# mpc001/auto_avsr

Measured on AMD Instinct MI355X. Metric: video-frames/sec/node (25fps 88x88, max-frames=1600), E2E training step (fwd+bwd+clip+AdamW), higher is better.
Workload: dtype f16 activations x f16x2 weights (atrunk3, atrunk4, decoder, encoder, trunk3, trunk4) + split-bf16 (everything else) forward / bf16 backward

## Files before the change

### auto_avsr_amd/csrc/gemm_core.h

```cpp
#pragma once
#include <algorithm>
#include "prims.h"

namespace avsr_gemm_impl {

struct Params {
    const void* A;
    const void* B;
    const void* B2;
    int lda, ldb;
    int M, N, K;
    int k_chunk;
    const float* bias;
    int act;
    const void* gate;
    int gate_dtype, ldg;
    float gate_scale;
    float drop_p;
    uint64_t seed;
    float alpha;
    const float* alpha_dev;
    const uint64_t* seed_dev;
    const float* resid;
    int ldr;
    void* C;
    void* C2;
    int ldc2;
    int c_dtype, ldc;
    int accumulate;
    int nsplit, batch_h, nbatch;
    long sAb, sAh, sBb, sBh, sCb, sCh;
    int a_skew, skew_off, skew_lim;
    int resid_dtype;
    int cH, cW, cC;
    int cOH, cOW;
    int cKH, cKW, cS, cPH, cPW;
    int cT, cKT, cPT;
    float* colsum;
    float* colstat;
    int colstat_rows;
    float* colsum_a;
    int cN, xcd_order, ncls;
    int k_rot;
    int cls_tile0[5], cls_py[4], cls_px[4], cls_y0[4], cls_x0[4], cls_h[4], cls_w[4], cls_nkh[4], cls_nkw[4];
};

template <class T> struct Raw8;
template <> struct Raw8<bf16_t> {
    bf16x8 v;
    AVSR_DEV void zero() { v = bf16x8{0, 0, 0, 0, 0, 0, 0, 0}; }
    AVSR_DEV void load(const bf16_t* p) { v = *reinterpret_cast<const bf16x8*>(p); }
    AVSR_DEV void set(int e, const bf16_t* p) { v[e] = (short)*p; }
    AVSR_DEV float get(int e) const { return bf2f((bf16_t)v[e]); }
};
template <> struct Raw8<float> {
    f32x4 a, b;
    AVSR_DEV void zero() { a = f32x4{0, 0, 0, 0}; b = a; }
    AVSR_DEV void load(const float* p) {
        a = *reinterpret_cast<const f32x4*>(p);
        b = *reinterpret_cast<const f32x4*>(p + 4);
    }
    AVSR_DEV void set(int e, const float* p) {
        if (e < 4) a[e] = *p; else b[e - 4] = *p;
    }
    AVSR_DEV float get(int e) const { return e < 4 ? a[e] : b[e - 4]; }
};

template <class T>
AVSR_DEV Raw8<T> load_chunk(const T* base, int ld, int r, int c, int r_lim, int c_lim) {
    Raw8<T> out;
    if (r < r_lim && c + 8 <= c_lim) {
        out.load(base + (size_t)r * ld + c);
    } else {
        out.zero();
        if (r < r_lim) {
            for (int e = 0; e < 8; e++)
                if (c + e < c_lim) out.set(e, base + (size_t)r * ld + c + e);
        }
    }
    return out;
}

template <class T>
AVSR_DEV Raw8<T> load_chunk_skew(const T* base, int ld, int r, int c, int r_lim, int m_lim, int off, int lim) {
    Raw8<T> out;
    out.zero();
    if (r < r_lim) {
        for (int e = 0; e < 8; e++) {
            const int j = c + e + r - off;
            if (c + e < m_lim && j >= 0 && j < lim) out.set(e, base + (size_t)r * ld + j);
        }
    }
    return out;
}

template <int TM, int TN>
AVSR_DEV void epilogue(f32x16 (&acc)[TM][TN], const Params& p, int row0, int col0, int lane, int zs, long c_off) {
    const float inv_keep = p.drop_p > 0.f ? 1.0f / (1.0f - p.drop_p) : 1.0f;
    const float alpha = p.alpha * (p.alpha_dev ? *p.alpha_dev : 1.f);
    const uint64_t seed = p.seed + (p.seed_dev ? *p.seed_dev : 0ull);
#pragma unroll
    for (int i = 0; i < TM; i++)
#pragma unroll
        for (int j = 0; j < TN; j++) {
            const int col = col0 + j * 32 + (lane & 31);
            if (col >= p.N) continue;
            const float bias = (p.bias && zs == 0) ? p.bias[col] : 0.f;
#pragma unroll
            for (int r = 0; r < 16; r++) {
                const int row = row0 + i * 32 + (r & 3) + 8 * (r >> 2) + 4 * (lane >> 5);
                if (row >= p.M) continue;
                float v = acc[i][j][r] + bias;
                if (p.act == 1) v = fmaxf(v, 0.f);
                else if (p.act == 2) v = avsr_silu(v);
                if (p.gate) {
                    const float g = p.gate_dtype == 0
                                        ? reinterpret_cast<const float*>(p.gate)[(size_t)row * p.ldg + col]
                                        : bf2f(reinterpret_cast<const bf16_t*>(p.gate)[(size_t)row * p.ldg + col]);
                    v = g > 0.f ? v * p.gate_scale : 0.f;
                }
                if (p.drop_p > 0.f)
                    v *= dropout_scale(seed, (uint64_t)row * (uint64_t)p.N + col, p.drop_p, inv_keep);
                v *= alpha;
                if (p.resid && zs == 0)
                    v += p.resid_dtype == 0 ? p.resid[(size_t)row * p.ldr + col]
                                            : bf2f(reinterpret_cast<const bf16_t*>(p.resid)[(size_t)row * p.ldr + col]);
                if (p.c_dtype == 0) {
                    float* c = reinterpret_cast<float*>(p.C) + c_off + (size_t)row * p.ldc + col;
// ... 494 lines not shown
```

### auto_avsr_amd/csrc/gemm_fast.hip

```cpp
#include "gemm_fast_kernel.h"
#include "gemm_pair.h"
#include "avsr_hip.h"

namespace {

using avsr_gemm_impl::Params;

#define g_tune avsr_tune_knobs

using avsr_fast::FastKernel;

template <int BM, int BN, int STAGES, int CV, int WGM, int WGN, int ABL, int KS, int F16 = 0, int WP = 1>
__global__ __launch_bounds__(64 * WGM * WGN * KS) void gemm_fast_kernel(Params p) {
    AVSR_DYN_SMEM(smem);
    FastKernel<BM, BN, STAGES, CV, WGM, WGN, ABL, KS, F16, WP>::run(p, smem);
}

template <int BM, int BN, int STAGES, int CV = 0, int WGM = 2, int WGN = 2, int ABL = 0, int KS = 1, int F16 = 0, int WP = 1>
void launch_fast(Params& p, int split_k, hipStream_t stream) {
    using K = FastKernel<BM, BN, STAGES, CV, WGM, WGN, ABL, KS, F16, WP>;
    p.k_rot = CV == 0 ? g_tune[7] : 0;
    p.xcd_order = g_tune[1] == 0 ? (CV == 0 && BM == 64 && BN == 64) : (g_tune[1] == 1);
    int gy;
    if (CV == 0) {
        int kc = (p.K + split_k - 1) / split_k;
        kc = ((kc + 63) / 64) * 64;
        split_k = (p.K + kc - 1) / kc;
        p.k_chunk = kc;
        gy = (p.M + BM - 1) / BM;
    } else {
        split_k = 1;
        int t0 = 0;
        for (int c = 0; c < p.ncls; c++) {
            p.cls_tile0[c] = t0;
            t0 += (int)(((long)p.cN * p.cls_h[c] * p.cls_w[c] + BM - 1) / BM);
        }
        p.cls_tile0[p.ncls] = t0;
        gy = t0;
    }
    dim3 grid((p.N + BN - 1) / BN, gy, split_k), block(K::NTHR);
    AVSR_LAUNCH((gemm_fast_kernel<BM, BN, STAGES, CV, WGM, WGN, ABL, KS, F16, WP>), grid, block, K::LDS_BYTES, stream, p);
}

template <int CV>
bool launch_tile(int tile, Params& p, int split_k, hipStream_t stream) {
    switch (tile) {
        case 1: if (CV == 0) { launch_fast<64, 64, 3, 0>(p, split_k, stream); return true; } return false;
        case 2: launch_fast<128, 64, 3, CV>(p, split_k, stream); return true;
        case 3:
            if (CV == 1 && g_tune[2] == 1) launch_fast<128, 128, 3, 1, 2, 2, 1>(p, split_k, stream);
            else if (CV == 1 && g_tune[2] == 2) launch_fast<128, 128, 3, 1, 2, 2, 2>(p, split_k, stream);
            else launch_fast<128, 128, 3, CV>(p, split_k, stream);
            return true;
        case 4: launch_fast<128, 128, 2, CV>(p, split_k, stream); return true;
        case 5: launch_fast<256, 128, 3, CV, 4, 2>(p, split_k, stream); return true;
        case 6: launch_fast<256, 128, 3, CV, 2, 2>(p, split_k, stream); return true;
        case 7: launch_fast<128, 64, 2, CV>(p, split_k, stream); return true;
        case 8: launch_fast<256, 64, 3, CV, 4, 2>(p, split_k, stream); return true;
        case 9: if (CV == 0) { launch_fast<64, 64, 5, 0>(p, split_k, stream); return true; } return false;
        case 10: if (CV == 0) { launch_fast<64, 64, 8, 0>(p, split_k, stream); return true; } return false;
        case 11: if (CV == 0) { launch_fast<128, 64, 4, 0>(p, split_k, stream); return true; } return false;
        case 12: if (CV == 0) { launch_fast<128, 64, 6, 0>(p, split_k, stream); return true; } return false;
        case 13: if (CV == 0) { launch_fast<128, 128, 4, 0>(p, split_k, stream); return true; } return false;
        case 14: if (CV == 0) { launch_fast<64, 64, 3, 0, 2, 2, 1>(p, split_k, stream); return true; } return false;
        case 15: if (CV == 0) { launch_fast<64, 64, 3, 0, 2, 2, 2>(p, split_k, stream); return true; } return false;
        case 16: if (CV == 0) { launch_fast<64, 64, 3, 0, 2, 2, 0, 2>(p, split_k, stream); return true; } return false;
        case 17: if (CV == 0) { launch_fast<128, 64, 3, 0, 2, 2, 0, 2>(p, split_k, stream); return true; } return false;
        case 18: if (CV == 0) { launch_fast<128, 128, 3, 0, 2, 2, 0, 2>(p, split_k, stream); return true; } return false;
        default: return false;
    }
}

template <int CV>
bool launch_tile_h16(int tile, Params& p, int split_k, hipStream_t stream) {
    switch (tile) {
        case 1: if (CV == 0) { launch_fast<64, 64, 3, 0, 2, 2, 0, 1, 1>(p, split_k, stream); return true; } return false;
        case 4: launch_fast<128, 128, 2, CV, 2, 2, 0, 1, 1>(p, split_k, stream); return true;
        case 7: launch_fast<128, 64, 2, CV, 2, 2, 0, 1, 1>(p, split_k, stream); return true;
        default: return false;
    }
}

template <int CV>
bool launch_tile_h16x2(int tile, Params& p, int split_k, hipStream_t stream) {
    switch (tile) {
        case 1: if (CV == 0) { launch_fast<64, 64, 3, 0, 2, 2, 0, 1, 1, 2>(p, split_k, stream); return true; } return false;
        case 21: if (CV == 0) { launch_fast<64, 64, 2, 0, 2, 2, 0, 1, 1, 2>(p, split_k, stream); return true; } return false;
        case 4: launch_fast<128, 128, 2, CV, 2, 2, 0, 1, 1, 2>(p, split_k, stream); return true;
        case 7: launch_fast<128, 64, 2, CV, 2, 2, 0, 1, 1, 2>(p, split_k, stream); return true;
        case 2: launch_fast<128, 64, 3, CV, 2, 2, 0, 1, 1, 2>(p, split_k, stream); return true;
        case 5: launch_fast<256, 128, 2, CV, 4, 2, 0, 1, 1, 2>(p, split_k, stream); return true;
        case 8: launch_fast<256, 64, 2, CV, 4, 2, 0, 1, 1, 2>(p, split_k, stream); return true;
        case 22: launch_fast<128, 128, 2, CV, 2, 4, 0, 1, 1, 2>(p, split_k, stream); return true;
        case 23: launch_fast<256, 64, 3, CV, 4, 2, 0, 1, 1, 2>(p, split_k, stream); return true;
        case 31: if (CV == 0) { launch_fast<64, 64, 3, 0, 2, 2, 1, 1, 1, 2>(p, split_k, stream); return true; } return false;
        case 32: if (CV == 0) { launch_fast<64, 64, 3, 0, 2, 2, 2, 1, 1, 2>(p, split_k, stream); return true; } return false;
        case 33: if (CV == 0) { launch_fast<128, 64, 2, 0, 2, 2, 1, 1, 1, 2>(p, split_k, stream); return true; } return false;
        case 34: if (CV == 0) { launch_fast<128, 64, 2, 0, 2, 2, 2, 1, 1, 2>(p, split_k, stream); return true; } return false;
        case 35: if (CV == 0) { launch_fast<256, 128, 2, 0, 4, 2, 1, 1, 1, 2>(p, split_k, stream); return true; } return false;
        case 36: if (CV == 0) { launch_fast<256, 128, 2, 0, 4, 2, 2, 1, 1, 2>(p, split_k, stream); return true; } return false;
        default: return false;
    }
}

}

int avsr_conv_patch_supported(int N, int H, int W, int Cg, int Cout_eff, int KH, int KW, int stride, int pad_h, int pad_w);
int avsr_conv_patch_launch(int mode, const void* src, const void* w, const void* w_lo, int ldw, const void* resid, void* out, void* out2,
                           const void* zero_page, int N, int H, int W, int Cg, int Cout_eff, hipStream_t stream);
int avsr_conv3x3_c64_supported(int H, int W);
int avsr_conv3x3_c64_launch(int flip, const void* src, const void* wq, const void* resid, void* out, const void* zero_page, int N,
                            int H, int W, hipStream_t stream);

static int gemm16_nt_impl(int f16, const void* A, int lda, const void* B, const void* B_lo, int ldb, int M, int N, int K, const float* bias,
                          int act, const void* gate, int gate_dtype, int ldg, float gate_scale, float drop_p,
                          uint64_t seed, const uint64_t* seed_dev, float alpha, const float* alpha_dev,
                          const void* resid, int resid_dtype, int ldr, void* C, int c_dtype, int ldc, int accumulate,
                          int split_k, int tile, float* colsum, void* c2, int ldc2, hipStream_t stream) {
    AVSR_REQUIRE(!(colsum && accumulate), "gemm_bf16_nt: colsum needs a non-accumulating output");
    AVSR_REQUIRE(K > 0 && K % 64 == 0, "gemm_bf16_nt: K must be a positive multiple of 64");
    AVSR_REQUIRE(lda % 8 == 0 && ldb % 8 == 0, "gemm_bf16_nt: lda/ldb must be multiples of 8 elements");
    AVSR_REQUIRE(((uintptr_t)A % 16) == 0 && ((uintptr_t)B % 16) == 0, "gemm_bf16_nt: operands must be 16-byte aligned");
    AVSR_REQUIRE(!(accumulate && c_dtype != 0), "gemm_bf16_nt: accumulate needs an f32 output");
// ... 371 lines not shown
```

### auto_avsr_amd/csrc/gemm_fast_kernel.h

```cpp
#pragma once
#include <type_traits>
#include "gemm_core.h"

namespace avsr_fast {

using avsr_gemm_impl::Params;

template <int BM, int BN, int STAGES, int CV = 0, int WGM = 2, int WGN = 2, int ABL = 0, int KS = 1, int F16 = 0, int WP = 1>
struct FastKernel {
    static_assert(WP == 1 || (WP == 2 && F16 == 1 && KS == 1), "two weight planes: f16 operands only");
    static constexpr int BK = 64, NQ = WGM * WGN, NW = NQ * KS, NTHR = 64 * NW;
    static constexpr int KPG = (BK / 16) / KS;
    static_assert(KS == 1 || KS == 2 || KS == 4, "k-split of the 64-wide tile");
    static constexpr int WM = BM / WGM, WN = BN / WGN, TM = WM / 32, TN = WN / 32;
    static constexpr int A_BYTES = BM * 128, B_BYTES = BN * 128, STAGE_BYTES = A_BYTES + WP * B_BYTES;
    static constexpr int A_LOADS = BM / (8 * NW), B_LOADS = BN / (8 * NW);
    static constexpr int LPT = A_LOADS + WP * B_LOADS;
    static constexpr size_t RING_BYTES = (size_t)STAGES * STAGE_BYTES, EPI_BYTES = (size_t)BM * (BN + 4) * 4;
    static constexpr size_t MAP_OFF = RING_BYTES > EPI_BYTES ? RING_BYTES : EPI_BYTES;
    static constexpr size_t LDS_BYTES = MAP_OFF + (CV == 2 ? BM * 4 : 0);
    static_assert(A_LOADS >= 1 && B_LOADS >= 1 && BM % (8 * NW) == 0 && BN % (8 * NW) == 0, "tile / wave-count mismatch");
    static_assert(WM % 32 == 0 && WN % 32 == 0, "wave tile must be a multiple of 32x32");

    struct Rows {
// ... 30 lines not shown
            if (CV == 0) {
                const int gr = min(m0 + r, p.M - 1);
                ri.a[i] = A + (size_t)gr * p.lda + c * 8;
                ri.mask[i] = 0;
            } else {
                int n, a, b;
                row_coords(p, cls, m0 + r, n, a, b);
                int ya, xa;
                if (CV == 1) {
                    ya = a * p.cS - p.cPH;
                    xa = b * p.cS - p.cPW;
                } else {
                    ya = (p.cls_y0[cls] + a * p.cS + p.cPH) / p.cS;
                    xa = (p.cls_x0[cls] + b * p.cS + p.cPW) / p.cS;
                }
                ri.a[i] = A + ((long)n * p.cH * p.cW + (long)ya * p.cW + xa) * p.cC + c * 8;
                uint32_t mk = 0;
                for (int t = 0; t < tp.ntaps; t++) {
                    const int ta = t / tp.nkw, tb = t - ta * tp.nkw;
                    const int y = CV == 1 ? ya + ta : ya - ta, x = CV == 1 ? xa + tb : xa - tb;
                    if (y >= 0 && y < p.cH && x >= 0 && x < p.cW) mk |= 1u << t;
                }
                ri.mask[i] = mk;
            }
        }
#pragma unroll
        for (int i = 0; i < B_LOADS; i++) {
            const int r = (wave * B_LOADS + i) * 8 + rsub;
            const int c = pc ^ ((r >> 1) & 7);
            const int gr = min(n0 + r, p.N - 1);
            ri.b[i] = B + (size_t)gr * p.ldb + c * 8;
        }
        return ri;
    }

    static AVSR_DEV void issue(const Params& p, const Rows& ri, const Taps& tp, int kbeg, int t, char* stage, int wave,
                               int rot = 0, int nt = 1) {
        long da, db;
        int tap = 0;
        if (CV == 0) {
            int tt = t + rot;
            if (tt >= nt) tt -= nt;
            da = db = kbeg + tt * BK;
        } else {
            tap = t / tp.cpt;
            const int cb = (t - tap * tp.cpt) * BK;
            const int ta = tap / tp.nkw, tb = tap - ta * tp.nkw;
            if (CV == 1) {
                da = (long)(ta * p.cW + tb) * p.cC + cb;
                db = (long)tap * p.cC + cb;
            } else {
                da = -(long)(ta * p.cW + tb) * p.cC + cb;
                db = (long)((tp.py + ta * p.cS) * p.cKW + tp.px + tb * p.cS) * p.cC + cb;
            }
        }
#pragma unroll
        for (int i = 0; i < A_LOADS; i++) {
            const bf16_t* src = ri.a[i] + da;
            if (CV != 0) src = ((ri.mask[i] >> tap) & 1u) ? src : reinterpret_cast<const bf16_t*>(p.gate);
            glds16(src, stage + (wave * A_LOADS + i) * 1024);
        }
#pragma unroll
        for (int i = 0; i < B_LOADS; i++) glds16(ri.b[i] + db, stage + A_BYTES + (wave * B_LOADS + i) * 1024);
        if (WP == 2) {
            const long lo = reinterpret_cast<const bf16_t*>(p.B2) - reinterpret_cast<const bf16_t*>(p.B);
#pragma unroll
            for (int i = 0; i < B_LOADS; i++) glds16(ri.b[i] + db + lo, stage + A_BYTES + B_BYTES + (wave * B_LOADS + i) * 1024);
        }
    }

    static AVSR_DEV bf16x8 frag(const char* base, int r, int chunk) {
        return *reinterpret_cast<const bf16x8*>(base + r * 128 + ((chunk ^ ((r >> 1) & 7)) << 4));
    }

    static AVSR_DEV void run(const Params& p, char* smem) {
        run_at(p, smem, blockIdx.x, blockIdx.y, blockIdx.z, gridDim.x, gridDim.y, gridDim.z);
    }
    static AVSR_DEV void run_at(const Params& p, char* smem, int bx, int by, int bz, int gx_, int gy_, int gz_) {
        const bf16_t* A = reinterpret_cast<const bf16_t*>(p.A);
        const bf16_t* B = reinterpret_cast<const bf16_t*>(p.B);
        const int lane = threadIdx.x & 63, wave = wave_id();
        const int kg = wave / NQ, wq = wave - kg * NQ;
        const int wm = wq / WGN, wn = wq % WGN;
        if (p.xcd_order && gz_ == 1) {
            const int gx = gx_, total = gx * gy_;
            const int id = by * gx + bx;
            const int xcd = id & 7, slot = id >> 3, q = total >> 3, r = total & 7;
            const int nid = (xcd < r ? xcd * (q + 1) : r * (q + 1) + (xcd - r) * q) + slot;
            by = nid / gx;
            bx = nid - by * gx;
        }
        const int n0 = bx * BN;
        const int zs = bz;

        int cls = 0, m0 = by * BM, nt, kbeg = 0;
        Taps tp{1, 1, 1, 0, 0};
        if (CV == 0) {
            kbeg = zs * p.k_chunk;
            nt = (min(p.K, kbeg + p.k_chunk) - kbeg) / BK;
        } else {
            while (cls + 1 < p.ncls && by >= p.cls_tile0[cls + 1]) cls++;
            m0 = (by - p.cls_tile0[cls]) * BM;
            tp.nkw = p.cls_nkw[cls];
            tp.ntaps = p.cls_nkh[cls] * tp.nkw;
            tp.cpt = p.cC / BK;
            tp.py = p.cls_py[cls];
            tp.px = p.cls_px[cls];
            nt = tp.ntaps * tp.cpt;
        }
        int* rowmap = nullptr;
        if (CV == 2) {
            rowmap = reinterpret_cast<int*>(smem + MAP_OFF);
            for (int r = threadIdx.x; r < BM; r += NTHR) {
                int n, a, b;
                const bool ok = row_coords(p, cls, m0 + r, n, a, b);
                rowmap[r] = ok ? (n * p.cOH + p.cls_y0[cls] + a * p.cS) * p.cOW + p.cls_x0[cls] + b * p.cS : -1;
            }
        }

        f32x16 acc[TM][TN];
        f32x16 acc_lo[WP == 2 ? TM : 1][WP == 2 ? TN : 1];
#pragma unroll
        for (int i = 0; i < TM; i++)
#pragma unroll
            for (int j = 0; j < TN; j++)
#pragma unroll
                for (int r = 0; r < 16; r++) {
                    acc[i][j][r] = 0.f;
                    if (WP == 2) acc_lo[i][j][r] = 0.f;
                }

        const Rows ri = decode_rows(p, A, B, m0, n0, cls, tp, wave, lane);
        const int rot = (CV == 0 && p.k_rot) ? (int)(((unsigned)(by * gx_ + bx) * (unsigned)p.k_rot) % (unsigned)nt) : 0;
#pragma unroll
        for (int s = 0; s < STAGES - 1; s++)
            if (s < nt) issue(p, ri, tp, kbeg, s, smem + s * STAGE_BYTES, wave, rot, nt);

        auto step = [&](int t, auto issue_flag) {
            constexpr bool ISSUE = decltype(issue_flag)::value;
            if (ISSUE) {
                wait_vmcnt<(STAGES - 2) * LPT>();
            } else {
                switch (nt - 1 - t) {
                    case 0: wait_vmcnt<0>(); break;
                    default: wait_vmcnt<(STAGES > 2 ? LPT : 0)>(); break;
                }
            }
            block_barrier_raw();
            const char* As = smem + (t % STAGES) * STAGE_BYTES;
            const char* Bs = As + A_BYTES;
            bf16x8 fa[2][TM], fb[2][TN], fl[2][WP == 2 ? TN : 1];
            const int arow = wm * WM + (lane & 31), brow = wn * WN + (lane & 31);
            auto load_frags = [&](int set, int ks) {
                const int chunk = ks * 2 + (lane >> 5);
#pragma unroll
                for (int i = 0; i < TM; i++) fa[set][i] = frag(As, arow + i * 32, chunk);
#pragma unroll
                for (int j = 0; j < TN; j++) fb[set][j] = frag(Bs, brow + j * 32, chunk);
                if (WP == 2) {
#pragma unroll
                    for (int j = 0; j < TN; j++) fl[set][j] = frag(Bs + B_BYTES, brow + j * 32, chunk);
                }
            };
            const int ks0 = kg * KPG;
            if (ABL != 1) {
                load_frags(0, ks0);
                if (KPG > 1) load_frags(1, ks0 + 1);
// ... 42 lines not shown
```

### auto_avsr_amd/csrc/gemm_pair.hip

```cpp
#include "gemm_fast_kernel.h"
#include "gemm_tn_kernel.h"
#include "gemm_pair.h"
#include "avsr_hip.h"

namespace {

using avsr_gemm_impl::Params;
using avsr_fast::FastKernel;
using Tn = avsr_tn::TnKernel<3, 0>;
using Tn4 = avsr_tn::TnKernel<3, 0, 1, 1, 4>;
using Tn128 = avsr_tn::TnKernel<2, 0, 2, 2>;

struct PairState {
    bool active = false, have_nt = false, have_tn = false;
    Params nt, tn;
    int nt_tile = 0;
    int gxa = 0, gya = 0;
    int gxb = 0, gyb = 0, gzb = 0;
    int tn_big = 0;
    hipStream_t stream = nullptr;
};
thread_local PairState g_pair;

template <class KA, class KB>
__global__ __launch_bounds__(256) void gemm_pair_kernel(Params pa, Params pb, int na, int gxa, int gya, int gxb, int gyb) {
    AVSR_DYN_SMEM(smem);
    int b = blockIdx.x;
    if (b < na) {
        const int by = b / gxa;
        KA::run_at(pa, smem, b - by * gxa, by, 0, gxa, gya, 1);
    } else {
        b -= na;
        const int r = b / gxb;
        KB::run_at(pb, smem, b - r * gxb, r % gyb, r / gyb);
    }
}

template <class KA, class KB>
void launch_pair(const PairState& s) {
    const int na = s.have_nt ? s.gxa * s.gya : 0;
    const int nb = s.have_tn ? s.gxb * s.gyb * s.gzb : 0;
    const size_t lds = KA::LDS_BYTES > KB::LDS_BYTES ? KA::LDS_BYTES : KB::LDS_BYTES;
    AVSR_LAUNCH((gemm_pair_kernel<KA, KB>), dim3(na + nb), dim3(256), lds, s.stream, s.nt, s.tn, na, s.gxa > 0 ? s.gxa : 1,
                s.gya > 0 ? s.gya : 1, s.gxb > 0 ? s.gxb : 1, s.gyb > 0 ? s.gyb : 1);
}

}

namespace avsr_pair {

bool stash_nt(const Params& p, int tile, int split_k, hipStream_t stream) {
    PairState& s = g_pair;
    if (!s.active || s.have_nt || split_k > 1 || p.accumulate || (tile != 1 && tile != 7)) return false;
    if (s.have_tn && s.stream != stream) return false;
    s.nt = p;
    s.nt.xcd_order = (tile == 1 && avsr_tune_knobs[1] != 2) ? 1 : 0;
    s.nt.k_chunk = ((p.K + 63) / 64) * 64;
    s.nt_tile = tile;
    const int BM = tile == 1 ? 64 : 128;
    s.gxa = (p.N + 63) / 64;
    s.gya = (p.M + BM - 1) / BM;
    s.stream = stream;
    s.have_nt = true;
    return true;
}

bool stash_tn(const Params& p, int split_k, hipStream_t stream) {
    PairState& s = g_pair;
    if (!s.active || s.have_tn) return false;
    if (s.have_nt && s.stream != stream) return false;
    if (split_k < 1) split_k = 1;
    int kc = (p.K + split_k - 1) / split_k;
    kc = ((kc + 63) / 64) * 64;
    split_k = (p.K + kc - 1) / kc;
    s.tn = p;
    s.tn_big = avsr_tune_knobs[19] == 2 && p.M >= 128 && p.N >= 128;
    if (s.tn_big) {
        split_k = 1;
        kc = ((p.K + 63) / 64) * 64;
    }
    const int tb = s.tn_big ? 128 : 64;
    s.tn.k_chunk = kc;
    s.gxb = (p.N + tb - 1) / tb;
    s.gyb = (p.M + tb - 1) / tb;
    s.gzb = split_k;
    s.stream = stream;
    s.have_tn = true;
    return true;
}

}

extern "C" int avsr_gemm_pair_begin(void) {
    AVSR_REQUIRE(!g_pair.active, "gemm_pair_begin: a pair is already open on this thread");
    g_pair = PairState{};
    g_pair.active = true;
    return 0;
}

extern "C" int avsr_gemm_pair_end(void) {
    PairState s = g_pair;
    g_pair = PairState{};
    AVSR_REQUIRE(s.active, "gemm_pair_end: no open pair on this thread");
    if (!s.have_nt && !s.have_tn) return 0;
    if (s.tn_big) {
        if (s.have_nt && s.nt_tile == 7) launch_pair<FastKernel<128, 64, 2, 0>, Tn128>(s);
        else launch_pair<FastKernel<64, 64, 3, 0>, Tn128>(s);
    } else if (avsr_tune_knobs[20] == 1) {
        if (s.have_nt && s.nt_tile == 7) launch_pair<FastKernel<128, 64, 2, 0>, Tn4>(s);
        else launch_pair<FastKernel<64, 64, 3, 0>, Tn4>(s);
    } else if (s.have_nt && s.nt_tile == 7) launch_pair<FastKernel<128, 64, 2, 0>, Tn>(s);
    else launch_pair<FastKernel<64, 64, 3, 0>, Tn>(s);
    AVSR_CHECK_LAUNCH("gemm_pair");
    return 0;
}
```

### auto_avsr_amd/csrc/gemm_tn_fast.hip

```cpp
#include "gemm_tn_kernel.h"
#include "gemm_pair.h"
#include "avsr_hip.h"

namespace {

using avsr_gemm_impl::Params;

using avsr_tn::TnKernel;

template <int STAGES, int CV>
__global__ __launch_bounds__(256) void gemm_tn_fast_kernel(Params p) {
    AVSR_DYN_SMEM(smem);
    TnKernel<STAGES, CV>::run(p, smem);
}

template <int CV>
void launch_tn(Params& p, int split_k, hipStream_t stream) {
    if (split_k < 1) split_k = 1;
    int kc = (p.K + split_k - 1) / split_k;
    kc = ((kc + 63) / 64) * 64;
    split_k = (p.K + kc - 1) / kc;
    p.k_chunk = kc;
    dim3 grid((p.N + 63) / 64, (p.M + 63) / 64, split_k), block(256);
    AVSR_LAUNCH((gemm_tn_fast_kernel<3, CV>), grid, block, (TnKernel<3, CV>::LDS_BYTES), stream, p);
}

}

extern "C" int avsr_gemm_bf16_tn(const void* A, int lda, const void* B, int ldb, int M, int N, int K, float* C, int ldc,
                                 int accumulate, int split_k, const void* zero_page, float* colsum_a, hipStream_t stream) {
    AVSR_REQUIRE(lda % 8 == 0 && ldb % 8 == 0 && M % 8 == 0 && N % 8 == 0, "gemm_bf16_tn: M, N, lda, ldb must be multiples of 8");
    AVSR_REQUIRE(((uintptr_t)A % 16) == 0 && ((uintptr_t)B % 16) == 0, "gemm_bf16_tn: operands must be 16-byte aligned");
    AVSR_REQUIRE(zero_page != nullptr, "gemm_bf16_tn: zero page required");
    AVSR_REQUIRE(!(split_k > 1 && !accumulate), "gemm_bf16_tn: split-K needs accumulate=1");
    if (M <= 0 || N <= 0 || K <= 0) return 0;
    Params p{};
    p.A = A; p.B = B; p.lda = lda; p.ldb = ldb; p.M = M; p.N = N; p.K = K;
    p.alpha = 1.f; p.gate_scale = 1.f; p.gate = zero_page;
    p.C = C; p.c_dtype = 0; p.ldc = ldc; p.accumulate = accumulate;
    p.colsum_a = colsum_a;
    p.nsplit = 1; p.batch_h = 1; p.nbatch = 1;
    if (avsr_det()) {
        p.colsum_a = nullptr;
        launch_tn<0>(p, 1, stream);
        if (colsum_a) avsr_colsum_det(A, 1, lda, K, M, colsum_a, stream);
        AVSR_CHECK_LAUNCH("gemm_bf16_tn");
        return 0;
    }
    if (avsr_pair::stash_tn(p, split_k, stream)) return 0;
    launch_tn<0>(p, split_k, stream);
    AVSR_CHECK_LAUNCH("gemm_bf16_tn");
    return 0;
}

extern "C" int avsr_conv2d_wgrad_bf16(const void* dy, const void* x, float* dwp, const void* zero_page, int N, int H, int W,
                                      int Cin, int Cout, int KH, int KW, int stride, int pad_h, int pad_w,
                                      hipStream_t stream) {
    AVSR_REQUIRE(Cin % 64 == 0 && Cout % 8 == 0, "conv2d_wgrad_bf16: Cin must be a multiple of 64, Cout of 8");
    AVSR_REQUIRE(zero_page != nullptr, "conv2d_wgrad_bf16: zero page required");
    const int OH = (H + 2 * pad_h - KH) / stride + 1, OW = (W + 2 * pad_w - KW) / stride + 1;
    if (N <= 0) return 0;
    Params p{};
    p.A = dy; p.B = x; p.lda = Cout; p.ldb = Cin;
    p.M = Cout; p.N = KH * KW * Cin; p.K = N * OH * OW;
    p.alpha = 1.f; p.gate_scale = 1.f; p.gate = zero_page;
    p.C = dwp; p.c_dtype = 0; p.ldc = p.N; p.accumulate = 1;
    p.nsplit = 1; p.batch_h = 1; p.nbatch = 1;
    p.cH = H; p.cW = W; p.cC = Cin; p.cOH = OH; p.cOW = OW; p.cKH = KH; p.cKW = KW; p.cS = stride; p.cPH = pad_h; p.cPW = pad_w;
    p.cT = 1; p.cKT = 1;
    const long tiles = (long)((p.M + 63) / 64) * ((p.N + 63) / 64);
    const long target = avsr_tune_knobs[24] > 0 ? avsr_tune_knobs[24] : (tiles <= 12 ? 512 : (tiles >= 96 ? 2048 : 1024));
    long split = target / (tiles < 1 ? 1 : tiles);
    if (split > p.K / 512) split = p.K / 512;
    if (split < 1 || avsr_det()) split = 1;
    launch_tn<3>(p, (int)split, stream);
    AVSR_CHECK_LAUNCH("conv2d_wgrad_bf16");
    return 0;
}
```

### auto_avsr_amd/csrc/gemm_tn_kernel.h

```cpp
#pragma once
#include "gemm_core.h"

namespace avsr_tn {

using avsr_gemm_impl::Params;

template <int STAGES, int CV, int TMS = 1, int TNS = 1, int DEPTH = 2>
struct TnKernel {
    static_assert(DEPTH == 2 || DEPTH == 4, "fragment pipeline depth");
    static_assert(CV == 0 || (TMS == 1 && TNS == 1), "gathered B operand: 64 x 64 tiles only");
    static constexpr int BM = 64 * TMS, BN = 64 * TNS, BK = 64;
    static constexpr int OP_BYTES = BK * 128;
    static constexpr int A_BYTES = TMS * OP_BYTES, STAGE_BYTES = (TMS + TNS) * OP_BYTES;
    static constexpr int LPT = 2 * (TMS + TNS);
    static constexpr size_t RING_BYTES = (size_t)STAGES * STAGE_BYTES, EPI_BYTES = (size_t)BM * (BN + 4) * 4;
    static constexpr size_t LDS_BYTES = RING_BYTES > EPI_BYTES ? RING_BYTES : EPI_BYTES;

    static AVSR_DEV void issue(const Params& p, const bf16_t* A, const bf16_t* B, int m0, int n0, int k0, int kend,
                               char* stage, int wave, int lane) {
        const int ksub = lane >> 3, chunk = (lane & 7) * 8;
        const bf16_t* zero = reinterpret_cast<const bf16_t*>(p.gate);
        int kh = 0, kw = 0, cbase = 0;
        if (CV == 3) {
            const int tap = n0 / p.cC;
            cbase = n0 - tap * p.cC;
            kh = tap / p.cKW;
            kw = tap - kh * p.cKW;
        }
#pragma unroll
        for (int i = 0; i < 2; i++) {
            const int kr = (wave * 2 + i) * 8 + ksub;
            const int k = k0 + kr;
            const bool kin = k < kend;
#pragma unroll
            for (int s = 0; s < TMS; s++) {
                const int mc = m0 + s * 64 + chunk;
                const bf16_t* sa = (kin && mc < p.M) ? A + (size_t)k * p.lda + mc : zero;
                glds16(sa, stage + s * OP_BYTES + (wave * 2 + i) * 1024);
            }
#pragma unroll
            for (int s = 0; s < TNS; s++) {
                const bf16_t* sb = zero;
                if (CV == 0) {
                    const int nc = n0 + s * 64 + chunk;
                    if (kin && nc < p.N) sb = B + (size_t)k * p.ldb + nc;
                } else if (kin) {
                    const int pix = p.cOH * p.cOW;
                    const int n = k / pix, r = k - n * pix;
                    const int oh = r / p.cOW, ow = r - oh * p.cOW;
                    const int ih = oh * p.cS + kh - p.cPH, iw = ow * p.cS + kw - p.cPW;
                    if (ih >= 0 && ih < p.cH && iw >= 0 && iw < p.cW)
                        sb = B + (((size_t)n * p.cH + ih) * p.cW + iw) * p.cC + cbase + chunk;
                }
                glds16(sb, stage + A_BYTES + s * OP_BYTES + (wave * 2 + i) * 1024);
            }
        }
    }

    static AVSR_DEV void frag_async(const char* base, int c0, int ks, int lane, bf16x4& lo, bf16x4& hi) {
        const int g = lane >> 4, i = lane & 15;
        const bf16_t* t = reinterpret_cast<const bf16_t*>(base);
        const int row = ks * 16 + 8 * (g >> 1) + (i >> 2);
        const int col = c0 + 16 * (g & 1) + 4 * (i & 3);
        lo = lds_tr16_async(t + row * 64 + col);
        hi = lds_tr16_async(t + (row + 4) * 64 + col);
    }

    static AVSR_DEV void run(const Params& p, char* smem) { run_at(p, smem, blockIdx.x, blockIdx.y, blockIdx.z); }
    static AVSR_DEV void run_at(const Params& p, char* smem, int bx, int by, int bz) {
        const bf16_t* A = reinterpret_cast<const bf16_t*>(p.A);
        const bf16_t* B = reinterpret_cast<const bf16_t*>(p.B);
        const int lane = threadIdx.x & 63, wave = wave_id();
        const int wm = wave >> 1, wn = wave & 1;
        const int m0 = by * BM, n0 = bx * BN;
        const int zs = bz;
        const int kbeg = zs * p.k_chunk;
        const int kend = min(p.K, kbeg + p.k_chunk);
        const int nt = (kend - kbeg + BK - 1) / BK;
        f32x16 acc[TMS][TNS];
#pragma unroll
        for (int i = 0; i < TMS; i++)
#pragma unroll
            for (int j = 0; j < TNS; j++)
#pragma unroll
                for (int r = 0; r < 16; r++) acc[i][j][r] = 0.f;
        const bool do_cs = CV == 0 && p.colsum_a != nullptr && bx == 0;
        float cs[TMS];
#pragma unroll
        for (int s = 0; s < TMS; s++) cs[s] = 0.f;
#pragma unroll
        for (int s = 0; s < STAGES - 1; s++)
            if (s < nt) issue(p, A, B, m0, n0, kbeg + s * BK, kend, smem + s * STAGE_BYTES, wave, lane);
        constexpr int NF = 2 * (TMS + TNS);
        for (int t = 0; t < nt; t++) {
            const int later = min(STAGES - 2, nt - 1 - t);
            if (later >= 1) wait_vmcnt<LPT>(); else wait_vmcnt<0>();
            block_barrier_raw();
            if (t + STAGES - 1 < nt)
                issue(p, A, B, m0, n0, kbeg + (t + STAGES - 1) * BK, kend, smem + ((t + STAGES - 1) % STAGES) * STAGE_BYTES,
                      wave, lane);
            const char* As = smem + (t % STAGES) * STAGE_BYTES;
            const char* Bs = As + A_BYTES;
            if (do_cs) {
#pragma unroll
                for (int s = 0; s < TMS; s++) {
                    const bf16_t* col = reinterpret_cast<const bf16_t*>(As + s * OP_BYTES) + (wave * 16) * 64 + lane;
#pragma unroll
                    for (int r = 0; r < 16; r++) cs[s] += bf2f(col[r * 64]);
                }
            }
            bf16x4 fa[DEPTH][TMS][2], fb[DEPTH][TNS][2];
            auto request = [&](int set, int ks) {
#pragma unroll
                for (int i = 0; i < TMS; i++) {
                    const int col = wm * 32 * TMS + 32 * i;
                    frag_async(As + (col >> 6) * OP_BYTES, col & 63, ks, lane, fa[set][i][0], fa[set][i][1]);
                }
#pragma unroll
                for (int j = 0; j < TNS; j++) {
                    const int col = wn * 32 * TNS + 32 * j;
                    frag_async(Bs + (col >> 6) * OP_BYTES, col & 63, ks, lane, fb[set][j][0], fb[set][j][1]);
                }
            };
            request(0, 0);
            if (DEPTH == 4) {
#pragma unroll
                for (int ks = 1; ks < BK / 16; ks++) request(ks, ks);
            }
#pragma unroll
            for (int ks = 0; ks < BK / 16; ks++) {
                const int c = DEPTH == 4 ? ks : (ks & 1);
                if (DEPTH == 4) {
                    switch (ks) {
                        case 0: lds_wait<3 * NF>(); break;
                        case 1: lds_wait<2 * NF>(); break;
                        case 2: lds_wait<NF>(); break;
                        default: lds_wait<0>(); break;
                    }
                } else if (ks + 1 < BK / 16) {
                    request(c ^ 1, ks + 1);
                    lds_wait<NF>();
                } else {
                    lds_wait<0>();
                }
                bf16x8 a[TMS], b[TNS];
#pragma unroll
                for (int i = 0; i < TMS; i++) {
                    lds_tie(fa[c][i][0]);
                    lds_tie(fa[c][i][1]);
                    a[i] = bf16x8{fa[c][i][0][0], fa[c][i][0][1], fa[c][i][0][2], fa[c][i][0][3],
                                  fa[c][i][1][0], fa[c][i][1][1], fa[c][i][1][2], fa[c][i][1][3]};
                }
// ... 27 lines not shown
```

### include/avsr_hip.h

```cpp
#ifndef AVSR_HIP_H
#define AVSR_HIP_H
#include <stdint.h>

#if defined(__HIP__) || defined(AVSR_EMU)
typedef hipStream_t avsr_stream_t;
#else
typedef void* avsr_stream_t;
#endif

#ifdef __cplusplus
extern "C" {
#endif

int avsr_abi_version(void);
int avsr_is_emulator(void);
const char* avsr_last_error(void);

int avsr_layernorm_fwd(const float* x, const float* gamma, const float* beta, void* y, int y_dtype,
                       float* mean, float* rstd, int rows, int cols, float eps,
                       avsr_stream_t stream);
int avsr_layernorm_fwd2(const float* x, const float* gamma, const float* beta, float* y, void* y2, float* mean, float* rstd,
                        int rows, int cols, float eps, avsr_stream_t stream);
int avsr_layernorm_bwd(const void* dy, int dy_dtype, const float* x, const float* gamma,
                       const float* mean, const float* rstd, const float* dres, float* dx,
// ... 153 lines not shown
int avsr_conv2d_fwd(const void* x, int dtype, const void* wp, int w_dtype, void* y, int N, int H, int W, int Cin,
                    int Cout, int KH, int KW, int stride, int pad_h, int pad_w, int precise, avsr_stream_t stream);
int avsr_conv2d_dgrad(const void* dy, int dtype, const void* wpd, int w_dtype, const void* resid, void* dx, int N,
                      int H, int W, int Cin, int Cout, int KH, int KW, int stride, int pad_h, int pad_w, int precise,
                      avsr_stream_t stream);
int avsr_conv2d_wgrad(const void* dy, const void* x, int dtype, float* dwp, int N, int H, int W, int Cin, int Cout,
                      int KH, int KW, int stride, int pad_h, int pad_w, int precise, avsr_stream_t stream);
int avsr_conv_stem_fwd(const float* x, const void* wp, int w_dtype, int ldw, void* y, int y_dtype, int B, int T, int H,
                       int W, int Cout, int KT, int KH, int KW, int stride, int pad_t, int pad_h, int pad_w,
                       int precise, avsr_stream_t stream);
int avsr_conv_stem_wgrad(const void* dy, int dy_dtype, const float* x, float* dw, int B, int T, int H, int W, int Cout,
                         int KT, int KH, int KW, int stride, int pad_t, int pad_h, int pad_w, int precise,
                         avsr_stream_t stream);

int avsr_maxpool2d_fwd(const void* x, void* y, uint8_t* idx, int dtype, int64_t N, int H, int W, int C, int K, int S, int P,
                       avsr_stream_t stream);
int avsr_maxpool2d_bwd(const uint8_t* idx, const void* dy, void* dx, int dtype, int64_t N, int H, int W, int C, int K, int S,
                       int P, avsr_stream_t stream);
int avsr_avgpool_fwd(const void* x, int dtype, float* y, int64_t groups, int win, int C, avsr_stream_t stream);
int avsr_avgpool_bwd(const float* dy, void* dx, int dtype, int64_t groups, int win, int C, avsr_stream_t stream);

int avsr_gemm_bf16_nt(const void* A, int lda, const void* B, int ldb, int M, int N, int K, const float* bias, int act,
                      const void* gate, int gate_dtype, int ldg, float gate_scale, float drop_p, uint64_t seed,
                      const uint64_t* seed_dev, float alpha, const float* alpha_dev, const void* resid, int resid_dtype,
                      int ldr, void* C, int c_dtype, int ldc, int accumulate, int split_k, int tile,
                      float* colsum ,
                      avsr_stream_t stream);
int avsr_gemm_f32s_nt(const float* A, int lda, const float* B, int ldb, int M, int N, int K, const float* bias, int act,
                      const void* gate, int gate_dtype, int ldg, float gate_scale, float drop_p, uint64_t seed,
                      const uint64_t* seed_dev, float alpha, const float* alpha_dev, const void* resid, int resid_dtype,
                      int ldr, void* C, int c_dtype, int ldc, int accumulate, int split_k, int tile, float* colsum,
                      int b_split ,
                      void* c2 , int ldc2,
                      avsr_stream_t stream);
int avsr_split_pack(const float* src, void* dst, int64_t n, avsr_stream_t stream);
int avsr_multi_split_pack(const void* table, int n, int total_blocks, avsr_stream_t stream);
int avsr_conv2d_f32s(const float* x, const float* wp, float* y, const void* zero_page, int N, int H, int W, int Cin, int Cout,
                     int KH, int KW, int stride, int pad_h, int pad_w, int tile, int w_split ,
                     void* y2 , avsr_stream_t stream);
int avsr_conv2d_f32s_stats(const float* x, const float* wp, float* y, const void* zero_page, int N, int H, int W, int Cin,
                           int Cout, int KH, int KW, int stride, int pad_h, int pad_w, int tile, int w_split, void* y2,
                           float* stats_part, int stats_tiles, avsr_stream_t stream);
int avsr_bn_finalize_parts(const float* part, int ntiles, int C, const float* zeros, float* ws, int64_t rows, float eps, float momentum,
                           float* mean, float* invstd, float* running_mean, float* running_var, int64_t* num_batches_tracked,
                           avsr_stream_t stream);
int avsr_bn_stats_parts(const float* part, int ntiles, int C, const float* zeros, float* ws, float* stats, float* count_out, int64_t rows,
                        avsr_stream_t stream);
int avsr_comm_unique_id(void* out128);
int avsr_comm_init(int slot, const void* id128, int nranks, int rank);
int avsr_comm_destroy(int slot);
int64_t avsr_comm_size(int slot);
int avsr_comm_all_reduce_f32(int slot, void* buf, int64_t count, avsr_stream_t stream);
int avsr_comm_all_reduce(int slot, void* buf, int64_t count, int dtype, avsr_stream_t stream);
int avsr_comm_all_gather_f32(int slot, const void* send, void* recv, int64_t count_per_rank, avsr_stream_t stream);
int avsr_comm_reduce_scatter(int slot, const void* send, void* recv, int64_t count_per_rank, int dtype, avsr_stream_t stream);
int avsr_tune(int knob, int value);
int avsr_conv2d_bf16(int dgrad, const void* src, const void* wp, const void* resid, void* out, const void* zero_page,
                     int N, int H, int W, int Cin, int Cout, int KH, int KW, int stride, int pad_h, int pad_w,
                     avsr_stream_t stream);
int avsr_transpose_cast(const void* src, int src_dtype, int64_t ld_src, void* dst, int64_t ld_dst, int R, int C,
                        avsr_stream_t stream);

int avsr_cast_transpose_colsum(const void* src, int src_dtype, int64_t ld_src, void* dst, void* dstT, int64_t ld_dstT,
                               float* colsum, int R, int C, float alpha, const float* alpha_dev, float drop_p,
                               uint64_t seed, const uint64_t* seed_dev, avsr_stream_t stream);

int avsr_multi_cast_transpose(const void* table, int n, int total_blocks, avsr_stream_t stream);

int64_t avsr_stem357_workspace_bytes(void);
int avsr_stem357_fwd(const float* x, const float* w, void* y, void* workspace, int B, int T, int H, int W,
                     avsr_stream_t stream);
int avsr_stem357_wgrad(const void* dy, const float* x, float* dw, void* workspace, int B, int T, int H, int W,
                       avsr_stream_t stream);
int avsr_stem357_fwd_f32s(const float* x, const float* w, float* y, void* y2 , void* workspace,
                          int B, int T, int H, int W, avsr_stream_t stream);
int64_t avsr_stem357_stat_rows(int B, int T, int H);
int avsr_stem357_fwd_f32s_stats(const float* x, const float* w, float* y, void* y2, void* workspace, int B, int T, int H, int W,
                                float* stats_part, int stats_rows, avsr_stream_t stream);

int avsr_gemm_bf16_tn(const void* A, int lda, const void* B, int ldb, int M, int N, int K, float* C, int ldc,
                      int accumulate, int split_k, const void* zero_page, float* colsum_a, avsr_stream_t stream);
int avsr_gemm_pair_begin(void);
int avsr_gemm_pair_end(void);
int avsr_conv2d_wgrad_bf16(const void* dy, const void* x, float* dwp, const void* zero_page, int N, int H, int W,
                           int Cin, int Cout, int KH, int KW, int stride, int pad_h, int pad_w,
                           avsr_stream_t stream);
int64_t avsr_conv3x3_wgrad_workspace_bytes(int N, int H, int W, int Cin, int Cout, int stride);
int avsr_conv3x3_wgrad_bf16(const void* dy, const void* x, float* dwp, const void* zero_page, void* workspace,
                            int64_t workspace_bytes, int N, int H, int W, int Cin, int Cout, int stride,
                            int torch_layout ,
                            avsr_stream_t stream);
int avsr_ctc_prefix_score(const float* logp, int T, int V, int ldv, const float* r_prev, const int64_t* last,
                          const int64_t* cand, int NH, int S, int out_len, int blank, float* r_new, float* psi,
                          float* psi_eos, avsr_stream_t stream);
int avsr_ctc_prefix_score_batch(int U, const float* const* logp, const int32_t* T, const int32_t* ldv, int V, const float* r_prev,
                                const int64_t* last, const int64_t* cand, const int32_t* row_off, const int32_t* n_rows,
                                const int64_t* frame_off, int pitch, int S, int out_len, int blank, float* r_new, float* psi,
                                float* psi_eos, avsr_stream_t stream);

int64_t avsr_beam_create(const int32_t* cfg, const float* fcfg, const void* const* w, int n_w);
int avsr_beam_destroy(int64_t handle);
int avsr_beam_attach_lm(int64_t handle, const int32_t* cfg, const float* fcfg, const void* const* w, int n_w);
#define AVSR_BIAS_MAX_NODES (1 << 24)
#define AVSR_BIAS_MAX_EDGES (1 << 24)
int avsr_bias_score(const int32_t* first, const int32_t* tok, const int32_t* child, const int32_t* unc, int n_nodes, int n_edges,
                    const int32_t* node, const int64_t* cand, int n, int S, int eos, float* gain, int32_t* next, avsr_stream_t stream);
int avsr_beam_set_bias(int64_t handle, const int32_t* cfg, const float* fcfg, const int32_t* first, const int32_t* tok,
                       const int32_t* child, const int32_t* unc);
int64_t avsr_beam_workspace_bytes(int64_t handle, int T, int Lmax);
int avsr_decode_linear(const float* A, int lda, const float* W, int M, int N, int K, const float* bias, const float* ln_g,
                       const float* ln_b, float eps, const float* st_in, int st_in_nt, int act, const float* resid, int ldr,
                       float* C, int ldc, float* st_out, int* st_out_nt, float* partial, avsr_stream_t stream);
int avsr_decode_attention(const float* q, int ldq, const float* kv, int64_t step_b, int64_t step_j, int koff, int voff, int n, int H,
                          int len, float* out, int ldo, int32_t* anc_scratch, avsr_stream_t stream);
int avsr_beam_begin(int64_t handle, const float* memory, int T, const float* ctc_logp, int ld_ctc, const float* r_init,
                    void* workspace, int64_t workspace_bytes, int Lmax, avsr_stream_t stream);
int avsr_beam_step(int64_t handle, float* host_out, int* n_out, avsr_stream_t stream);
int avsr_beam_keep(int64_t handle, const int32_t* keep, int n_keep, avsr_stream_t stream);
int avsr_beam_fetch_yseq(int64_t handle, int64_t* host_yseq, int* ldy_out, int* L_out, avsr_stream_t stream);
int64_t avsr_beam_batch_workspace_bytes(int64_t handle, int U, const int32_t* T, int Lmax);
int avsr_beam_begin_batch(int64_t handle, int U, const float* const* memory, const int32_t* T, const float* const* ctc_logp,
                          const int32_t* ld_ctc, const float* const* r_init, void* workspace, int64_t workspace_bytes, int Lmax,
                          avsr_stream_t stream);
int avsr_beam_step_batch(int64_t handle, float* host_out, int* n_out, avsr_stream_t stream);
int avsr_beam_keep_batch(int64_t handle, const int32_t* keep, const int32_t* n_keep, avsr_stream_t stream);
int avsr_beam_fetch_yseq_batch(int64_t handle, int64_t* host_yseq, int* ldy_out, int* L_out, avsr_stream_t stream);

int avsr_adamw_step(const void* table, int n, int total_blocks, float* partial, float* state, float base_lr, float beta1,
                    float beta2, float eps, float weight_decay, float max_grad_norm, int64_t warmup_steps,
                    int64_t total_steps, avsr_stream_t stream);
int avsr_multi_sumsq(const void* table, int n, int total_blocks, float* partial, float* sumsq, avsr_stream_t stream);
int avsr_adamw_apply(const void* table, int n, int total_blocks, const float* sumsq, float* state, float base_lr, float beta1,
                     float beta2, float eps, float weight_decay, float max_grad_norm, int64_t warmup_steps, int64_t total_steps,
                     avsr_stream_t stream);
int avsr_multi_copy_scale(const void* table, int n, int total_blocks, float scale, avsr_stream_t stream);
int avsr_adamw_cast_step(const void* table, int n, int total_blocks, const void* lin_table, int lin_n, int lin_blocks,
                         const void* tile_table, int tile_n, int tile_blocks, float* partial, float* state,
                         float base_lr, float beta1, float beta2, float eps, float weight_decay, float max_grad_norm,
                         int64_t warmup_steps, int64_t total_steps, avsr_stream_t stream);

int avsr_video_transform(const int64_t* src_ptr, const int32_t* lens, const int32_t* crop_y,
                         const int32_t* crop_x, const int32_t* iv, const int32_t* niv, int max_iv, void* out,
                         int out_dtype, int B, int Tmax, int H, int W, int crop, float mean, float std,
                         avsr_stream_t stream);
int64_t avsr_audio_transform_workspace_bytes(int B, int64_t Lmax);
int avsr_audio_transform(const int64_t* wav_ptr, const int32_t* lens, const int32_t* iv,
                         const int32_t* niv, int max_iv, const float* noise, const int64_t* noise_start,
                         const float* snr_db, float eps, float* out, int B, int64_t Lmax, void* workspace,
                         avsr_stream_t stream);

int avsr_layernorm_fwd_h16(const float* x, const float* gamma, const float* beta, void* y, void* y2, float* mean, float* rstd,
                           int rows, int cols, float eps, avsr_stream_t stream);
int avsr_gemm_h16_nt(const void* A, int lda, const void* B, const void* B_lo, int ldb, int M, int N, int K, const float* bias, int act,
                     float drop_p, uint64_t seed, const uint64_t* seed_dev, float alpha, const void* resid, int resid_dtype,
                     int ldr, void* C, int c_dtype, int ldc, int tile, void* c2, int ldc2, avsr_stream_t stream);
int avsr_conv2d_h16(const void* x, const void* wp, const void* wp_lo, int ldw, void* y, void* y2, const void* zero_page, int N, int H, int W, int Cin,
                    int Cout, int KH, int KW, int stride, int pad_h, int pad_w, avsr_stream_t stream);
int avsr_head_bias_fwd_h16(const void* x, int64_t ldx, const float* b1, const float* b2, void* o1, void* o2, void* t1, void* t2,
                           int64_t rows, int cols, avsr_stream_t stream);
int avsr_attention_fwd_h16(const void* qu, const void* qv, const void* k, const void* v, const void* pos, const uint8_t* mask,
                           int64_t mask_sb, int64_t mask_sq, void* out, void* out2, float* lse, int B, int H, int Tq, int Tk,
                           int dk, int ldq, int ldk, int ldv, int ldp, int ldo, int64_t sbq, int64_t sbk, int64_t sbv,
                           int64_t sbo, float scale, float drop_p, uint64_t seed, const uint64_t* seed_dev,
                           avsr_stream_t stream);
int avsr_dwconv_fwd_h16(const void* x, const float* w, const float* bias, void* y, void* y2, int B, int T, int C, int K,
                        int glu_in, avsr_stream_t stream);
// ... 11 lines not shown
```

Before: 70190.

## Partition GEMM tiles into per-XCD rectangular regions to improve L2 reuse

Adds a tile-remapping scheme that gives each of the eight XCDs a contiguous rectangular block of output tiles, optionally split along K. The split between M, N and K is chosen on the host by a cost model that minimises the A and B bytes each XCD must fetch. The remap is wired into the fast NT, TN and paired GEMM kernels, including an offset for the second GEMM inside a paired launch. Through a tuning-knob bitmask it is switched on by default only for the paired 64-wide NT GEMM. It adds some index arithmetic per block and may unbalance load when grid sizes do not divide evenly.

```diff
diff --git a/auto_avsr_amd/csrc/gemm_core.h b/auto_avsr_amd/csrc/gemm_core.h
--- a/auto_avsr_amd/csrc/gemm_core.h
+++ b/auto_avsr_amd/csrc/gemm_core.h
@@ -42,8 +42,77 @@
     float* colsum_a;
     int cN, xcd_order, ncls;
     int k_rot;
+    int xcd_part, xcd_off;
     int cls_tile0[5], cls_py[4], cls_px[4], cls_y0[4], cls_x0[4], cls_h[4], cls_w[4], cls_nkh[4], cls_nkw[4];
 };
+
+#define AVSR_HD __host__ __device__ __forceinline__
+
+AVSR_HD int xcd_pack(int lm, int ln, int lk) { return 64 | lm | (ln << 2) | (lk << 4); }
+
+AVSR_HD void xcd_cut(int& nid, int g, int l, int unit, int& lo, int& hi) {
+    for (int i = 0;; i++) {
+        lo = (i * g) >> l;
+        hi = ((i + 1) * g) >> l;
+        const int sz = (hi - lo) * unit;
+        if (nid < sz || i + 1 == (1 << l)) return;
+        nid -= sz;
+    }
+}
+
+AVSR_HD void xcd_tile_order(int b, int off, int gx, int gy, int gz, int part, int& bx, int& by, int& bz) {
+    const int lm = part & 3, ln = (part >> 2) & 3, lk = (part >> 4) & 3;
+    const int total = gx * gy * gz, q = total >> 3, r = total & 7, o = off & 7;
+    const int xcd = ((b & 7) + o) & 7, slot = b >> 3;
+    int extra = xcd - o;
+    extra = extra < 0 ? 0 : (extra > r ? r : extra);
+    if (extra > 8 - o) extra = 8 - o;
+    if (o + r > 8) extra += xcd < o + r - 8 ? xcd : o + r - 8;
+    int nid = xcd * q + extra + slot;
+    int z0, z1, y0, y1, x0, x1;
+    xcd_cut(nid, gz, lk, gx * gy, z0, z1);
+    const int hz = z1 - z0;
+    xcd_cut(nid, gy, lm, gx * hz, y0, y1);
+    const int hy = y1 - y0;
+    xcd_cut(nid, gx, ln, hy * hz, x0, x1);
+    const int hx = x1 - x0;
+    const int t = nid / hx, y = hz == 1 ? t : t % hy;
+    bx = x0 + nid - t * hx;
+    by = y0 + y;
+    bz = z0 + (hz == 1 ? 0 : t / hy);
+}
+
+inline int xcd_choose(int gx, int gy, int gz, int BM, int BN, int planes) {
+    long best = -1;
+    int best_part = xcd_pack(3, 0, 0);
+    for (int lk = 3; lk >= 0; lk--) {
+        if ((1 << lk) > gz) continue;
+        const int rest = 3 - lk;
+        for (int d = 0; d <= rest; d++) {
+            for (int s = 0; s < 2; s++) {
+                if ((rest - d) & 1) continue;
+                const int lm = s == 0 ? (rest + d) / 2 : (rest - d) / 2, ln = rest - lm;
+                if (s == 1 && d == 0) continue;
+                const long pm = std::min(1 << lm, gy), pn = std::min(1 << ln, gx);
+                const long cost = pn * gy * BM + pm * gx * BN * planes;
+                if (best < 0 || cost < best) {
+                    best = cost;
+                    best_part = xcd_pack(lm, ln, lk);
+                }
+            }
+        }
+    }
+    return best_part;
+}
+
+enum XcdFamily { XCD_NT_64 = 0, XCD_NT_WIDE = 1, XCD_PAIR_NT_64 = 2, XCD_PAIR_NT_128 = 3, XCD_TN = 4, XCD_PAIR_TN = 5, XCD_TN_GATHER = 6 };
+constexpr int XCD_ADOPTED = 1 << XCD_PAIR_NT_64;
+inline bool xcd_family_on(int family) {
+    const int k = avsr_tune_knobs[1];
+    if (k == 3) return true;
+    if (k == 1 || k == 2 || k == 4) return false;
+    return (((k >= 64 ? k - 64 : XCD_ADOPTED) >> family) & 1) != 0;
+}
 
 template <class T> struct Raw8;
 template <> struct Raw8<bf16_t> {
diff --git a/auto_avsr_amd/csrc/gemm_fast.hip b/auto_avsr_amd/csrc/gemm_fast.hip
--- a/auto_avsr_amd/csrc/gemm_fast.hip
+++ b/auto_avsr_amd/csrc/gemm_fast.hip
@@ -20,7 +20,7 @@
 void launch_fast(Params& p, int split_k, hipStream_t stream) {
     using K = FastKernel<BM, BN, STAGES, CV, WGM, WGN, ABL, KS, F16, WP>;
     p.k_rot = CV == 0 ? g_tune[7] : 0;
-    p.xcd_order = g_tune[1] == 0 ? (CV == 0 && BM == 64 && BN == 64) : (g_tune[1] == 1);
+    p.xcd_order = g_tune[1] == 1 ? 1 : (g_tune[1] == 2 ? 0 : (CV == 0 && BM == 64 && BN == 64));
     int gy;
     if (CV == 0) {
         int kc = (p.K + split_k - 1) / split_k;
@@ -39,6 +39,10 @@
         gy = t0;
     }
     dim3 grid((p.N + BN - 1) / BN, gy, split_k), block(K::NTHR);
+    p.xcd_off = 0;
+    p.xcd_part = 0;
+    if (CV == 0 && split_k == 1 && avsr_gemm_impl::xcd_family_on(BM == 64 && BN == 64 ? avsr_gemm_impl::XCD_NT_64 : avsr_gemm_impl::XCD_NT_WIDE))
+        p.xcd_part = avsr_gemm_impl::xcd_choose((int)grid.x, gy, 1, BM, BN, WP);
     AVSR_LAUNCH((gemm_fast_kernel<BM, BN, STAGES, CV, WGM, WGN, ABL, KS, F16, WP>), grid, block, K::LDS_BYTES, stream, p);
 }
 
diff --git a/auto_avsr_amd/csrc/gemm_fast_kernel.h b/auto_avsr_amd/csrc/gemm_fast_kernel.h
--- a/auto_avsr_amd/csrc/gemm_fast_kernel.h
+++ b/auto_avsr_amd/csrc/gemm_fast_kernel.h
@@ -136,7 +136,10 @@
         const int lane = threadIdx.x & 63, wave = wave_id();
         const int kg = wave / NQ, wq = wave - kg * NQ;
         const int wm = wq / WGN, wn = wq % WGN;
-        if (p.xcd_order && gz_ == 1) {
+        if (CV == 0 && p.xcd_part && gz_ == 1) {
+            int z;
+            avsr_gemm_impl::xcd_tile_order(by * gx_ + bx, p.xcd_off, gx_, gy_, 1, p.xcd_part, bx, by, z);
+        } else if (p.xcd_order && gz_ == 1) {
             const int gx = gx_, total = gx * gy_;
             const int id = by * gx + bx;
             const int xcd = id & 7, slot = id >> 3, q = total >> 3, r = total & 7;
diff --git a/auto_avsr_amd/csrc/gemm_pair.hip b/auto_avsr_amd/csrc/gemm_pair.hip
--- a/auto_avsr_amd/csrc/gemm_pair.hip
+++ b/auto_avsr_amd/csrc/gemm_pair.hip
@@ -32,7 +32,7 @@
     } else {
         b -= na;
         const int r = b / gxb;
-        KB::run_at(pb, smem, b - r * gxb, r % gyb, r / gyb);
+        KB::run_at(pb, smem, b - r * gxb, r % gyb, r / gyb, gxb, gyb, (int)(gridDim.x - na) / (gxb * gyb));
     }
 }
 
@@ -40,8 +40,11 @@
 void launch_pair(const PairState& s) {
     const int na = s.have_nt ? s.gxa * s.gya : 0;
     const int nb = s.have_tn ? s.gxb * s.gyb * s.gzb : 0;
+    PairState t = s;
+    t.nt.xcd_off = 0;
+    t.tn.xcd_off = na;
     const size_t lds = KA::LDS_BYTES > KB::LDS_BYTES ? KA::LDS_BYTES : KB::LDS_BYTES;
-    AVSR_LAUNCH((gemm_pair_kernel<KA, KB>), dim3(na + nb), dim3(256), lds, s.stream, s.nt, s.tn, na, s.gxa > 0 ? s.gxa : 1,
+    AVSR_LAUNCH((gemm_pair_kernel<KA, KB>), dim3(na + nb), dim3(256), lds, s.stream, t.nt, t.tn, na, s.gxa > 0 ? s.gxa : 1,
                 s.gya > 0 ? s.gya : 1, s.gxb > 0 ? s.gxb : 1, s.gyb > 0 ? s.gyb : 1);
 }
 
@@ -60,6 +63,8 @@
     const int BM = tile == 1 ? 64 : 128;
     s.gxa = (p.N + 63) / 64;
     s.gya = (p.M + BM - 1) / BM;
+    s.nt.xcd_part = avsr_gemm_impl::xcd_family_on(tile == 1 ? avsr_gemm_impl::XCD_PAIR_NT_64 : avsr_gemm_impl::XCD_PAIR_NT_128)
+                        ? avsr_gemm_impl::xcd_choose(s.gxa, s.gya, 1, BM, 64, 1) : 0;
     s.stream = stream;
     s.have_nt = true;
     return true;
@@ -84,6 +89,7 @@
     s.gxb = (p.N + tb - 1) / tb;
     s.gyb = (p.M + tb - 1) / tb;
     s.gzb = split_k;
+    s.tn.xcd_part = avsr_gemm_impl::xcd_family_on(avsr_gemm_impl::XCD_PAIR_TN) ? avsr_gemm_impl::xcd_choose(s.gxb, s.gyb, s.gzb, tb, tb, 1) : 0;
     s.stream = stream;
     s.have_tn = true;
     return true;
@@ -114,3 +120,23 @@
     AVSR_CHECK_LAUNCH("gemm_pair");
     return 0;
 }
+
+extern "C" int avsr_xcd_tile_order_host(int gx, int gy, int gz, int lm, int ln, int lk, int off, int* tile_of) {
+    AVSR_REQUIRE(gx > 0 && gy > 0 && gz > 0 && lm >= 0 && ln >= 0 && lk >= 0 && lm + ln + lk == 3 && (1 << lk) <= gz,
+                 "xcd_tile_order_host: the partition must have 8 regions and no more k ranges than k-splits");
+    const int total = gx * gy * gz;
+    for (int b = 0; b < total; b++) {
+        int bx, by, bz;
+        avsr_gemm_impl::xcd_tile_order(b, off, gx, gy, gz, avsr_gemm_impl::xcd_pack(lm, ln, lk), bx, by, bz);
+        tile_of[b] = (bz * gy + by) * gx + bx;
+    }
+    return 0;
+}
+
+extern "C" int avsr_xcd_choose_host(int gx, int gy, int gz, int bm, int bn, int planes, int* lmnk) {
+    const int part = avsr_gemm_impl::xcd_choose(gx, gy, gz, bm, bn, planes);
+    lmnk[0] = part & 3;
+    lmnk[1] = (part >> 2) & 3;
+    lmnk[2] = (part >> 4) & 3;
+    return 0;
+}
diff --git a/auto_avsr_amd/csrc/gemm_tn_fast.hip b/auto_avsr_amd/csrc/gemm_tn_fast.hip
--- a/auto_avsr_amd/csrc/gemm_tn_fast.hip
+++ b/auto_avsr_amd/csrc/gemm_tn_fast.hip
@@ -22,6 +22,9 @@
     split_k = (p.K + kc - 1) / kc;
     p.k_chunk = kc;
     dim3 grid((p.N + 63) / 64, (p.M + 63) / 64, split_k), block(256);
+    p.xcd_off = 0;
+    p.xcd_part = avsr_gemm_impl::xcd_family_on(CV == 0 ? avsr_gemm_impl::XCD_TN : avsr_gemm_impl::XCD_TN_GATHER)
+                     ? avsr_gemm_impl::xcd_choose((int)grid.x, (int)grid.y, split_k, 64, 64, 1) : 0;
     AVSR_LAUNCH((gemm_tn_fast_kernel<3, CV>), grid, block, (TnKernel<3, CV>::LDS_BYTES), stream, p);
 }
 
diff --git a/auto_avsr_amd/csrc/gemm_tn_kernel.h b/auto_avsr_amd/csrc/gemm_tn_kernel.h
--- a/auto_avsr_amd/csrc/gemm_tn_kernel.h
+++ b/auto_avsr_amd/csrc/gemm_tn_kernel.h
@@ -66,8 +66,11 @@
         hi = lds_tr16_async(t + (row + 4) * 64 + col);
     }
 
-    static AVSR_DEV void run(const Params& p, char* smem) { run_at(p, smem, blockIdx.x, blockIdx.y, blockIdx.z); }
-    static AVSR_DEV void run_at(const Params& p, char* smem, int bx, int by, int bz) {
+    static AVSR_DEV void run(const Params& p, char* smem) {
+        run_at(p, smem, blockIdx.x, blockIdx.y, blockIdx.z, gridDim.x, gridDim.y, gridDim.z);
+    }
+    static AVSR_DEV void run_at(const Params& p, char* smem, int bx, int by, int bz, int gx, int gy, int gz) {
+        if (p.xcd_part) avsr_gemm_impl::xcd_tile_order((bz * gy + by) * gx + bx, p.xcd_off, gx, gy, gz, p.xcd_part, bx, by, bz);
         const bf16_t* A = reinterpret_cast<const bf16_t*>(p.A);
         const bf16_t* B = reinterpret_cast<const bf16_t*>(p.B);
         const int lane = threadIdx.x & 63, wave = wave_id();
diff --git a/include/avsr_hip.h b/include/avsr_hip.h
--- a/include/avsr_hip.h
+++ b/include/avsr_hip.h
@@ -259,6 +259,8 @@
                       int accumulate, int split_k, const void* zero_page, float* colsum_a, avsr_stream_t stream);
 int avsr_gemm_pair_begin(void);
 int avsr_gemm_pair_end(void);
+int avsr_xcd_tile_order_host(int gx, int gy, int gz, int lm, int ln, int lk, int off, int* tile_of);
+int avsr_xcd_choose_host(int gx, int gy, int gz, int bm, int bn, int planes, int* lmnk);
 int avsr_conv2d_wgrad_bf16(const void* dy, const void* x, float* dwp, const void* zero_page, int N, int H, int W,
                            int Cin, int Cout, int KH, int KW, int stride, int pad_h, int pad_w,
                            avsr_stream_t stream);
```

Measured after the change: 70400 (median of 5 runs). About the same (+0.3%).
